# liannuaa/GenPC

Hardware: AMD Instinct MI355X
Metric: chamfer_nn_pair_dist_throughput (higher is better)
Workload: dtype f32; 1 GPU; chamfer_3DDist.forward B=1 N=M=16384 (both directions), one pair per rank; points=16384, batch=1, arith=fma

## Files before the change

### genpc_amd/csrc/chamfer.hip

```cpp
#include "nn.h"
#include "../../include/genpc_hip.h"

#include <stdlib.h>
#include <algorithm>
#include <atomic>
#include <mutex>

namespace genpc {

constexpr int kTile = 2048;




template <int R, int FMA>
__global__ __launch_bounds__(kBlock) void nn_forward_kernel(NNArgs a)
{
    __shared__ float4 tile[kTile / 4 * 3 + 3];
    const int lane = threadIdx.x & (kWave - 1);
    const int wave = threadIdx.x >> 6;
    int bid = blockIdx.x;
    const int d = (a.ndir > 1 && bid >= a.dir[1].block_begin) ? 1 : 0;
    const NNDir &D = a.dir[d];
    bid -= D.block_begin;
// ... 756 lines not shown
        NNDir &D = a.dir[d];
        D.slices = ceil_div(D.nt, a.slice_len);
        D.block_begin = (int)tb;
        D.unit_begin = units;
        tb += (long long)D.slices * b * D.qblocks;
        units += b * D.qblocks;
        if (D.slices > 1 || path == 2) {
            part += (size_t)D.slices * b * D.nq * pwords;
            any_split = true;
        }
    }
    if (tb > 0x7fffffffLL) {
        set_error("chamfer: problem too large for one launch");
        return 0;
    }
    if (any_split) {
        const size_t cnt_min = (size_t)1 << 16;
        size_t cnt_bytes = cnt_min;
        if ((size_t)units * sizeof(int) > cnt_bytes) cnt_bytes = ((size_t)units * sizeof(int) + 255) & ~(size_t)255;
        char *ws = (char *)workspace(0, cnt_bytes + part * 8, st, nullptr, cnt_min);
        if (!ws) return 0;
        if (cnt_bytes > cnt_min && !check(hipMemsetAsync(ws, 0, cnt_bytes, st), "hipMemsetAsync(arrival counters)")) return 0;
        a.arrive = (int *)ws;
        unsigned long long *wp = (unsigned long long *)(ws + cnt_bytes);
        size_t off = 0;
        for (int d = 0; d < nd; d++) {
            if (a.dir[d].slices > 1 || path == 2) {
                a.dir[d].part = wp + off;
                off += (size_t)a.dir[d].slices * b * a.dir[d].nq * pwords;
            }
        }
    }
    if (path == 2) {
        const int force = (a.debug & 2048) ? 0 : ((a.debug & 4096) ? 1 : -1);
        DedupeHint *H = dedupe_hint();
        bool own_masks = true;
        for (int d = 0; d < nd; d++) own_masks = own_masks && a.dir[d].dupmask != nullptr;
        if (force == 0) {
            for (int d = 0; d < nd; d++) a.dir[d].dupmask = nullptr;
        } else if (!own_masks) {
            long long queries = 0, targets = 0;
            for (int d = 0; d < nd; d++) { queries += (long long)b * a.dir[d].nq; targets += (long long)b * a.dir[d].nt; }
            bool run = force == 1;
            if (!run && H) {
                std::lock_guard<std::mutex> l(H->mu);
                volatile unsigned *hv = H->host;
// ... 116 lines not shown
```

### genpc_amd/csrc/nn.h

```cpp
#pragma once
#include "common.h"
#include "grid.h"

namespace genpc {

constexpr int kChunk = 32;
constexpr int kBlock = 256;
constexpr int kWavesPerBlock = kBlock / kWave;

template <int FMA>
__device__ __forceinline__ float sqdist(float dx, float dy, float dz)
{
    if (FMA) {
        float t = __fmul_rn(dy, dy);
        t = __fmaf_rn(dx, dx, t);
        return __fmaf_rn(dz, dz, t);
    } else {
        float a = __fmul_rn(dx, dx);
        float b = __fmul_rn(dy, dy);
        float c = __fmul_rn(dz, dz);
        return __fadd_rn(__fadd_rn(a, b), c);
    }
}

struct NNDir {
    const float *q;
    const float *t;
    float *out_d;
    int *out_i;
    unsigned long long *part;
    int nq, nt;
    float *tmaxp;
    const uint4 *arec;
    int ntp, ntmax;
    int fin_begin;
    const unsigned *dupmask;
    int dup_shared;
    int qblocks;
    int slices;
    int block_begin;
    int unit_begin;
};

struct NNArgs {
    NNDir dir[2];
    int ndir;
    int b;
    int slice_len;
    int *arrive;
    int debug;
    int fma;
    unsigned long long *stats;
    int hint_stride;
    unsigned *hint;
    float radius2;
};

typedef float f32x16 __attribute__((ext_vector_type(16)));

struct Top3 {
    float a1, a2, a3;
    int c1, c2;
};

__device__ __forceinline__ void top3_init(Top3 &s)
{
    s.a1 = s.a2 = s.a3 = __builtin_inff();
    s.c1 = s.c2 = -1;
}

__device__ __forceinline__ void top3_insert(Top3 &s, float m, int id)
{
    asm("v_cmp_lt_f32 vcc, %[m], %[a2]\n\t"
        "v_cndmask_b32 %[c2], %[c2], %[id], vcc\n\t"
        "v_cmp_lt_f32 vcc, %[m], %[a1]\n\t"
        "v_cndmask_b32 %[c2], %[c2], %[c1], vcc\n\t"
        "v_cndmask_b32 %[c1], %[c1], %[id], vcc\n\t"
        "v_med3_f32 %[a3], %[a2], %[a3], %[m]\n\t"
// ... 35 lines not shown
            for (int c = 7; c >= 0; c--) {
                const float dd = sqdist<FMA>(f[c * 3 + 0] - qx, f[c * 3 + 1] - qy, f[c * 3 + 2] - qz);
                const bool le = dd <= bd;
                bd = le ? dd : bd;
                bi = le ? base + c8 + c : bi;
            }
        }
    } else {
        for (int c = LEN - 1; c >= 0; c--) {
            int kk = base + c;
            kk = kk < nt ? kk : nt - 1;
            const float *tp = T + (size_t)kk * 3;
            const float dd = sqdist<FMA>(tp[0] - qx, tp[1] - qy, tp[2] - qz);
            const bool le = dd <= bd;
            bd = le ? dd : bd;
            bi = le ? kk : bi;
        }
    }
}

__device__ __forceinline__ int tile_row(int w) { return 8 * ((w >> 2) & 3) + 4 * (w >> 4) + (w & 3); }

constexpr int kRefTile = 512;
template <int FMA>
__device__ __forceinline__ void nn_exhaustive(const float *__restrict__ Qp, const float *__restrict__ T, int nt, int j,
                                              float *__restrict__ od, int *__restrict__ oi, float *s_red, int *s_fi)
{
    const int lane = threadIdx.x & (kWave - 1), wave = threadIdx.x >> 6;
    const float x = Qp[(size_t)j * 3 + 0], y = Qp[(size_t)j * 3 + 1], z = Qp[(size_t)j * 3 + 2];
    int dead = 0;
    for (int k = threadIdx.x * kRefTile; k < nt; k += kBlock * kRefTile) {
        const float *tp = T + (size_t)k * 3;
        const float hd = sqdist<FMA>(tp[0] - x, tp[1] - y, tp[2] - z);
        dead |= hd != hd;
    }
    dead = __syncthreads_or(dead);
    float bd = __builtin_inff();
    int bi = 0x7fffffff;
    if (!dead) {
        for (int k = threadIdx.x; k < nt; k += kBlock) {
            const float *tp = T + (size_t)k * 3;
            const float dd = sqdist<FMA>(tp[0] - x, tp[1] - y, tp[2] - z);
            const bool lt = dd < bd;
            bd = lt ? dd : bd;
            bi = lt ? k : bi;
        }
    } else {
        for (int k = threadIdx.x; k < nt; k += kBlock) {
            const float *hp = T + (size_t)(k & ~(kRefTile - 1)) * 3;
            const float hd = sqdist<FMA>(hp[0] - x, hp[1] - y, hp[2] - z);
            const float *tp = T + (size_t)k * 3;
            const float dd = sqdist<FMA>(tp[0] - x, tp[1] - y, tp[2] - z);
            const bool lt = dd < bd && hd == hd;
            bd = lt ? dd : bd;
            bi = lt ? k : bi;
        }
    }
#pragma unroll
    for (int o = 32; o >= 1; o >>= 1) {
        const float obd = __shfl_xor(bd, o);
        const int obi = __shfl_xor(bi, o);
        const bool other = obd < bd || (obd == bd && obi < bi);
        bd = other ? obd : bd;
        bi = other ? obi : bi;
    }
    __syncthreads();
    if (lane == 0) { s_red[wave] = bd; s_fi[wave] = bi; }
    __syncthreads();
    if (threadIdx.x == 0) {
        for (int w = 1; w < kWavesPerBlock; w++) {
            const bool other = s_red[w] < bd || (s_red[w] == bd && s_fi[w] < bi);
            bd = other ? s_red[w] : bd;
            bi = other ? s_fi[w] : bi;
        }
        const float d0 = sqdist<FMA>(T[0] - x, T[1] - y, T[2] - z);
        if (d0 != d0 || bi == 0x7fffffff) {
            bd = d0;
            bi = 0;
        }
        od[j] = bd;
        oi[j] = bi;
    }
}

__device__ __forceinline__ float nn_tau(float a_best, float qq, float tmax2, double kQT, double kTT)
{
    const double u = 1.01 * 5.9604644775390625e-8;
    const double T = sqrt((double)tmax2), qn = sqrt((double)qq);
    const double kSub = 64.0 * 1.401298464324817e-45;
    const double E1 = u * (kQT * qn * T + kTT * T * T + 3.0 * (double)qq) + kSub;
    const double eta = u * (qn + T);
    double up = (double)a_best + (double)qq + E1;
    up = sqrt(up > 0.0 ? up : 0.0) + eta;
// ... 26 lines not shown
            const float f[12] = {v[g * 3].x, v[g * 3].y, v[g * 3].z, v[g * 3].w, v[g * 3 + 1].x, v[g * 3 + 1].y,
                                 v[g * 3 + 1].z, v[g * 3 + 1].w, v[g * 3 + 2].x, v[g * 3 + 2].y, v[g * 3 + 2].z, v[g * 3 + 2].w};
#pragma unroll
            for (int c = 3; c >= 0; c--) {
                const float dd = sqdist<FMA>(f[c * 3 + 0] - qx, f[c * 3 + 1] - qy, f[c * 3 + 2] - qz);
                const bool le = dd <= bd;
                bd = le ? dd : bd;
                bi = le ? first + 4 * g + c : bi;
            }
        }
    } else {
        for (int c = 15; c >= 0; c--) {
            int kk = first + c;
            kk = kk < nt ? kk : nt - 1;
            const float *tp = T + (size_t)kk * 3;
            const float dd = sqdist<FMA>(tp[0] - qx, tp[1] - qy, tp[2] - qz);
            const bool le = dd <= bd;
            bd = le ? dd : bd;
            bi = le ? kk : bi;
        }
    }
}

int launch_nn_f16(NNArgs &a, int q, int u, int nl, int tight, long long total_blocks, hipStream_t st);
int launch_nn_finish(NNArgs &a, int nl, int upieces, float kqt, float ktt, float t2min, hipStream_t st);
int launch_nn_grid(const NNArgs &a, hipStream_t st);
size_t nn_dedupe_mask_words(int b, int n);
int launch_nn_dedupe(int b, int nclouds, const float *const pts[2], const int n[2], unsigned *const masks[2], unsigned *hint,
                     hipStream_t st);
int nn_forward(int b, int ndir, const float *q0, int n0, const float *t0, int m0, float *d0, int *i0, const float *q1,
               int n1, const float *t1, int m1, float *d1, int *i1, hipStream_t st, float radius2 = __builtin_inff(),
               const unsigned *dup0 = nullptr, const unsigned *dup1 = nullptr, int dup_shared = 0);

struct SeededGrids {
    const CellGridHdr *hdr_static, *hdr_rest;
    const int *start_static, *start_rest;
    const float4 *sorted_static, *sorted_rest;
};
size_t seeded_grids_bytes(int b, int nm, int ns);
int build_seeded_grids(int b, int nm, const float *rest_pts, int ns, const float *static_pts, void *ws, SeededGrids &g, hipStream_t st);
int launch_nn_seeded(int b, int nm, const float *moving_pts, int ns, const float *static_pts, const SeededGrids &g, const float *center,
                     int cstride, const float *params, int pstride, float *d1, int *i1, float *d2, int *i2, int fma, hipStream_t st, int sample = 1);

}
```

### genpc_amd/csrc/nn_f16.hip

```cpp
#include "nn.h"
#include <hip/hip_ext.h>
#include "../../include/genpc_hip.h"

#include <stdlib.h>

namespace genpc {

typedef _Float16 h16x8 __attribute__((ext_vector_type(8)));

#ifdef GENPC_NN_TIMELINE
__device__ unsigned long long g_timeline[4096 * 8];
#define GENPC_TL(k) do { if (threadIdx.x == 0 && blockIdx.x < 4096) { g_timeline[blockIdx.x * 8 + (k)] = __builtin_readcyclecounter(); \
    if ((k) == 0) g_timeline[blockIdx.x * 8 + 6] = wall_clock64(); if ((k) == 5) g_timeline[blockIdx.x * 8 + 7] = wall_clock64(); } } while (0)
#else
#define GENPC_TL(k) do {} while (0)
#endif
constexpr int kHTile = 1024;
constexpr double kQTh = 30.0, kTTh = 15.0;

__device__ __forceinline__ unsigned f16_bits(float v) { return (unsigned)__builtin_bit_cast(unsigned short, (_Float16)v); }

__device__ __forceinline__ unsigned split2(float v)
{
    const _Float16 h = (_Float16)v;
    const _Float16 l = (_Float16)(v - (float)h);
    return (unsigned)__builtin_bit_cast(unsigned short, h) | ((unsigned)__builtin_bit_cast(unsigned short, l) << 16);
}

__device__ __forceinline__ unsigned dup_lo(unsigned v) { return __builtin_amdgcn_perm(v, v, 0x01000100u); }
__device__ __forceinline__ unsigned dup_hi(unsigned v) { return __builtin_amdgcn_perm(v, v, 0x03020302u); }

__device__ __forceinline__ float scale_for(float m)
{
    if (!(m > 0.0f) || !(m < __builtin_inff())) return 1.0f;
    const int e = __builtin_amdgcn_frexp_expf(m);
    return __builtin_ldexpf(1.0f, 11 - e);
}

template <int Q, int U, int NL, int W, int HT, int WV>
__global__ __launch_bounds__(WV * kWave, W) void nn_f16_kernel(NNArgs a)
{
    constexpr int kThreads = WV * kWave;
    static_assert(Q >= 2, "one accumulator chain per wave violates the MFMA -> VALU wait states");
    constexpr int kC = 32 * U;
    constexpr int kRows = HT + 64;
    __shared__ uint4 plane[2][kRows];
    __shared__ float s_red[WV];
    GENPC_TL(0);
    const int lane = threadIdx.x & (kWave - 1);
    const int wave = threadIdx.x >> 6;
    const int half = lane >> 5, col = lane & 31;
    int bid = blockIdx.x;
    const int d = (a.ndir > 1 && bid >= a.dir[1].block_begin) ? 1 : 0;
    const NNDir &D = a.dir[d];
    bid -= D.block_begin;
    const int qb = bid % D.qblocks;
    const int rest = bid / D.qblocks;
    const int batch = rest % a.b;
    const int slice = rest / a.b;

    const int nq = D.nq, nt = D.nt;
    const float *__restrict__ Qp = D.q + (size_t)batch * nq * 3;
    const float *__restrict__ T = D.t + (size_t)batch * nt * 3;
    const float *cptr = a.dir[0].t + (size_t)batch * a.dir[0].nt * 3;
    const float cx = cptr[0], cy = cptr[1], cz = cptr[2];

    const int k_begin = slice * a.slice_len;
    int k_end = k_begin + a.slice_len;
    if (k_end > nt) k_end = nt;

// ... 132 lines not shown
                    float m[Q][4];
#pragma unroll
                    for (int r = 0; r < Q; r++) m[r][0] = m[r][1] = m[r][2] = m[r][3] = __builtin_inff();
#pragma unroll
                    for (int g = 0; g < U - 1; g++) {
                        if (g & 1) step(std::integral_constant<int, 1>{}, std::false_type{}, rb + 32 * g, m);
                        else step(std::integral_constant<int, 0>{}, std::false_type{}, rb + 32 * g, m);
                    }
                    if (rb + kC < tn_pad) step(std::integral_constant<int, 1>{}, std::false_type{}, rb + kC - 32, m);
                    else step(std::integral_constant<int, 1>{}, std::true_type{}, rb + kC - 32, m);
#pragma unroll
                    for (int r = 0; r < Q; r++) {
                        float v;
                        asm("v_min3_f32 %0, %1, %2, %3" : "=v"(v) : "v"(m[r][0]), "v"(m[r][1]), "v"(m[r][2]));
                        asm("v_min_f32 %0, %1, %2" : "=v"(v) : "v"(v), "v"(m[r][3]));
                        top3_insert(lst[r][n], v, t0 + rb + half);
                    }
                }
            }
        }
    }

    GENPC_TL(4);
    if (qb == 0) {
        if (nf != nf) tmax2 = __builtin_inff();
#pragma unroll
        for (int o = 32; o >= 1; o >>= 1) tmax2 = fmaxf(tmax2, __shfl_xor(tmax2, o));
        __syncthreads();
        if (lane == 0) s_red[wave] = tmax2;
        __syncthreads();
        float tm = s_red[0];
#pragma unroll
        for (int w2 = 1; w2 < WV; w2++) tm = fmaxf(tm, s_red[w2]);
        if (threadIdx.x == 0) D.tmaxp[(size_t)batch * D.slices + slice] = tm;
    }

    const size_t bnq = (size_t)a.b * nq;
    unsigned long long *P = D.part + (size_t)batch * nq;
#pragma unroll
    for (int r = 0; r < Q; r++) {
#pragma unroll
        for (int n = 0; n < NL; n++) {
            Top3 &f = lst[r][n];
            f.a1 = (f.a1 * isc) * isc;
            f.a2 = (f.a2 * isc) * isc;
            f.a3 = (f.a3 * isc) * isc;
            const float o1 = __shfl_xor(f.a1, 32), o2 = __shfl_xor(f.a2, 32), o3 = __shfl_xor(f.a3, 32);
            const int oc1 = __shfl_xor(f.c1, 32), oc2 = __shfl_xor(f.c2, 32);
            top3_insert(f, o1, oc1);
            top3_insert(f, o2, oc2);
            top3_insert(f, o3, -1);
            const int j = q0 + r * 32;
            if (!half && j < nq) {
                unsigned long long *p = P + (size_t)(slice * NL + n) * 2 * bnq + j;
                const unsigned code2 = list_enc(f.a1, f.a2);
                const unsigned code3 = list_enc(list_dec(f.a1, code2), f.a3);
                p[0] = ((unsigned long long)__float_as_uint(f.a1) << 32) | (unsigned)f.c1;
                p[bnq] = ((unsigned long long)((code2 << 16) | code3) << 32) | (unsigned)f.c2;
            }
        }
    }
    GENPC_TL(5);
}

template <int Q, int NL>
static void launch_main(const NNArgs &a, int blocks, int u, int tight, hipStream_t st, hipEvent_t e0 = nullptr, hipEvent_t e1 = nullptr)
{
#define NN_F16_LAUNCH(KERNEL, GRID, BLOCK)                                                                              \
    do {                                                                                                                \
        if (e0) hipExtLaunchKernelGGL(KERNEL, GRID, BLOCK, 0, st, e0, e1, 0, a);                                        \
        else hipLaunchKernelGGL(KERNEL, GRID, BLOCK, 0, st, a);                                                         \
    } while (0)
    const bool big = Q == 4 && tight != 1 && a.slice_len > kHTile;
    if (Q == 4 && tight == 2) {
        if (u == 2) NN_F16_LAUNCH((nn_f16_kernel<4, 2, NL, 1, 2 * kHTile, 8>), dim3(blocks), dim3(8 * kWave));
        else NN_F16_LAUNCH((nn_f16_kernel<4, 4, NL, 1, 2 * kHTile, 8>), dim3(blocks), dim3(8 * kWave));
        return;
    }
    if (big) {
        if (u == 2) NN_F16_LAUNCH((nn_f16_kernel<4, 2, NL, 2, 2 * kHTile, 4>), dim3(blocks), dim3(kBlock));
        else NN_F16_LAUNCH((nn_f16_kernel<4, 4, NL, 2, 2 * kHTile, 4>), dim3(blocks), dim3(kBlock));
        return;
    }
    if (u == 2) {
        if (tight) NN_F16_LAUNCH((nn_f16_kernel<Q, 2, NL, (Q == 4 ? 3 : 4), kHTile, 4>), dim3(blocks), dim3(kBlock));
        else NN_F16_LAUNCH((nn_f16_kernel<Q, 2, NL, (Q == 4 ? 2 : 4), kHTile, 4>), dim3(blocks), dim3(kBlock));
    } else {
        if (tight) NN_F16_LAUNCH((nn_f16_kernel<Q, 4, NL, (Q == 4 ? 3 : 4), kHTile, 4>), dim3(blocks), dim3(kBlock));
        else NN_F16_LAUNCH((nn_f16_kernel<Q, 4, NL, (Q == 4 ? 2 : 4), kHTile, 4>), dim3(blocks), dim3(kBlock));
    }
#undef NN_F16_LAUNCH
}

static thread_local bool g_prof_on = false;
static thread_local hipEvent_t g_prof_e0 = nullptr, g_prof_e1 = nullptr;

int launch_nn_f16(NNArgs &a, int q, int u, int nl, int tight, long long total_blocks, hipStream_t st)
{
    size_t bytes = 0;
    size_t off_t[2];
    for (int d = 0; d < a.ndir; d++) {
        a.dir[d].ntmax = a.dir[d].slices;
        off_t[d] = bytes;
        bytes += ((size_t)a.b * a.dir[d].ntmax * sizeof(float) + 255) & ~(size_t)255;
    }
    char *ws = (char *)workspace(9, bytes, st);
    if (!ws) return 0;
    for (int d = 0; d < a.ndir; d++) a.dir[d].tmaxp = (float *)(ws + off_t[d]);
    const int blocks = (int)total_blocks;
    hipEvent_t pe0 = nullptr, pe1 = nullptr;
    if (g_prof_on) {
        if (!g_prof_e0) { (void)hipEventCreate(&g_prof_e0); (void)hipEventCreate(&g_prof_e1); }
        pe0 = g_prof_e0;
        pe1 = g_prof_e1;
    }
    if (q == 4) {
        if (nl == 2) launch_main<4, 2>(a, blocks, u, tight, st, pe0, pe1);
        else launch_main<4, 1>(a, blocks, u, tight, st, pe0, pe1);
    } else {
        if (nl == 2) launch_main<2, 2>(a, blocks, u, 0, st, pe0, pe1);
        else launch_main<2, 1>(a, blocks, u, 0, st, pe0, pe1);
    }
    if (!check(hipGetLastError(), "nn_f16_kernel launch")) return 0;
    return launch_nn_finish(a, nl, u, (float)kQTh, (float)kTTh, 0.0f, st);
}

}

#ifdef GENPC_NN_TIMELINE
extern "C" __attribute__((visibility("default"))) int genpc_nn_timeline_read(unsigned long long *out)
{
    return hipMemcpyFromSymbol(out, HIP_SYMBOL(genpc::g_timeline), sizeof(unsigned long long) * 4096 * 8) == hipSuccess;
}
#endif

GENPC_API float genpc_nn_profile(int enable)
{
    using namespace genpc;
    float ms = -1.0f;
    if (g_prof_on && g_prof_e1 && hipEventSynchronize(g_prof_e1) == hipSuccess) (void)hipEventElapsedTime(&ms, g_prof_e0, g_prof_e1);
    g_prof_on = enable != 0;
    return ms;
}
```

### genpc_amd/csrc/nn_finish.hip

```cpp
#include "nn.h"

namespace genpc {

#ifdef GENPC_NN_TIMELINE
__device__ unsigned long long g_timeline_fin[4096 * 8];
#define GENPC_TLF(k) do { if (threadIdx.x == 0 && blockIdx.x < 4096) g_timeline_fin[blockIdx.x * 8 + (k)] = __builtin_readcyclecounter(); } while (0)
#else
#define GENPC_TLF(k) do {} while (0)
#endif

constexpr int kFQ = 64;
constexpr int kFWork = 2048;

template <int FMA>
__global__ __launch_bounds__(kBlock) void nn_finish_kernel(NNArgs a, int nl, int upieces, float kqt, float ktt, float t2min)
{
    __shared__ unsigned long long s_best[kFQ];
    __shared__ float4 s_q[kFQ];
    __shared__ float s_a[4][kFQ];
    __shared__ int s_c[4][kFQ];
    __shared__ int s_qflag[kFQ];
    __shared__ int s_flagged[kFQ];
    __shared__ unsigned s_work[kFWork];
    __shared__ float s_red[kWavesPerBlock];
    __shared__ int s_fi[kWavesPerBlock];
    __shared__ int s_misc[3];
    GENPC_TLF(0);
    const int lane = threadIdx.x & (kWave - 1), wave = threadIdx.x >> 6;
    int bid = blockIdx.x;
    const int d = (a.ndir > 1 && bid >= a.dir[1].fin_begin) ? 1 : 0;
    const NNDir &D = a.dir[d];
    bid -= D.fin_begin;
    const int nq = D.nq, nt = D.nt;
    const int fblocks = (nq + kFQ - 1) / kFQ;
    const int batch = bid / fblocks, fb = bid % fblocks;
    const float *__restrict__ Qp = D.q + (size_t)batch * nq * 3;
    const float *__restrict__ T = D.t + (size_t)batch * nt * 3;
    float *__restrict__ od = D.out_d + (size_t)batch * nq;
    int *__restrict__ oi = D.out_i + (size_t)batch * nq;
    const size_t bnq = (size_t)a.b * nq;
    const unsigned long long *P = D.part + (size_t)batch * nq;
    const int nlists = D.slices * nl;

    const int ql = threadIdx.x & (kFQ - 1), part = threadIdx.x >> 6;
    int j = fb * kFQ + ql;
    const bool live = j < nq;
    j = live ? j : nq - 1;

    const float *cptr = a.dir[0].t + (size_t)batch * a.dir[0].nt * 3;
    const float ccx = cptr[0], ccy = cptr[1], ccz = cptr[2];
    unsigned long long w0[kMaxLists / 4], w1[kMaxLists / 4];
    float amin = __builtin_inff();
#pragma unroll
    for (int k = 0; k < kMaxLists / 4; k++) {
        const int li = part + 4 * k;
        w0[k] = 0x7f800000ull << 32;
        w1[k] = 0xff00ff00ull << 32;
        if (li < nlists) {
            const unsigned long long *p = P + (size_t)li * 2 * bnq + j;
            w0[k] = p[0];
            w1[k] = p[bnq];
        }
    }
    int cmin = -1, kmin = -1;
#pragma unroll
    for (int k = 0; k < kMaxLists / 4; k++) {
        const float a1 = __uint_as_float((unsigned)(w0[k] >> 32));
        if (a1 < amin) { amin = a1; cmin = (int)(unsigned)w0[k]; kmin = k; }
    }
    s_a[part][ql] = amin;
    s_c[part][ql] = cmin;
    float tmax2 = 0.0f;
    {
        const float *tp = D.tmaxp + (size_t)batch * D.ntmax;
        for (int i = threadIdx.x; i < D.ntmax; i += kBlock) tmax2 = fmaxf(tmax2, tp[i]);
#pragma unroll
        for (int o = 32; o >= 1; o >>= 1) tmax2 = fmaxf(tmax2, __shfl_xor(tmax2, o));
        if (lane == 0) s_red[wave] = tmax2;
    }
    if (part == 0) {
        s_q[ql] = make_float4(Qp[(size_t)j * 3 + 0], Qp[(size_t)j * 3 + 1], Qp[(size_t)j * 3 + 2], 0.0f);
        s_best[ql] = ~0ull;
        s_qflag[ql] = 0;
    }
    if (threadIdx.x == 0) { s_misc[0] = 0; s_misc[1] = 0; s_misc[2] = 0; }
    __syncthreads();
    GENPC_TLF(1);
    tmax2 = fmaxf(fmaxf(s_red[0], s_red[1]), fmaxf(s_red[2], s_red[3]));
    int bp = 0;
    float abest = s_a[0][ql];
#pragma unroll
    for (int q2 = 1; q2 < 4; q2++) {
        const float v = s_a[q2][ql];
        if (v < abest) { abest = v; bp = q2; }
    }
    const int cb = s_c[bp][ql];
    const float4 qv = s_q[ql];
    unsigned long long mine = ~0ull;
    int pieces = 0;
    if (cb >= 0 && live && !(a.debug & 1)) {
        const int h = cb & 1, c0 = cb & ~1;
        const int left = (nt - c0 + 31) >> 5;
        const int n2 = left < upieces ? left : upieces;
        if (part < n2) {
            float dd;
            int ii;
            rescan_half<FMA>(T, nt, c0 + 32 * part, h, qv.x, qv.y, qv.z, dd, ii);
            mine = ((unsigned long long)__float_as_uint(dd) << 32) | (unsigned)ii;
            pieces = 1;
        }
    }
    float tau, qq;
    {
        const float x = qv.x - ccx, y = qv.y - ccy, z = qv.z - ccz;
        qq = __fmaf_rn(z, z, __fmaf_rn(y, y, __fmul_rn(x, x)));
        tau = nn_tau(abest, qq, tmax2, (double)kqt, (double)ktt);
        if (!(tmax2 >= t2min)) tau = __builtin_nanf("");
        if (!(tmax2 < __builtin_inff()) || !(qq < __builtin_inff())) tau = __builtin_nanf("");
        if (a.debug & 16) tau = __builtin_inff();
    }
    if (mine != ~0ull) atomicMin(&s_best[ql], mine);
    GENPC_TLF(2);
    bool flag = (a.debug & 8) != 0 || !(tau == tau);
    int ncand = 0;
    auto consider = [&](float av, int c, bool is_best) {
        if (av <= tau) {
            ncand++;
            if (c < 0) {
                flag = true;
            } else if (live && !is_best) {
                const int h = c & 1, c0 = c & ~1;
                const int left = (nt - c0 + 31) >> 5;
                const int n2 = left < upieces ? left : upieces;
                const int w = atomicAdd(&s_misc[0], n2);
                if (w + n2 <= kFWork) {
                    for (int k = 0; k < n2; k++) s_work[w + k] = ((unsigned)ql << 22) | (unsigned)((((c0 >> 5) + k) << 1) | h);
                } else {
                    flag = true;
                }
            }
        }
    };
#pragma unroll
    for (int k = 0; k < kMaxLists / 4; k++) {
        const float a1 = __uint_as_float((unsigned)(w0[k] >> 32));
        const unsigned codes = (unsigned)(w1[k] >> 32);
        const float a2 = list_dec(a1, codes >> 16), a3 = list_dec(a2, codes & 0xffffu);
        if (!(a3 > tau)) flag = true;
        consider(a1, (int)(unsigned)w0[k], part == bp && k == kmin);
        consider(a2, (int)(unsigned)w1[k], false);
    }
    if (flag && live) s_qflag[ql] = 1;
    if (a.debug & 32) {
        __syncthreads();
        if (part == 0) s_a[0][ql] = 0.0f;
        __syncthreads();
        atomicAdd(&s_a[0][ql], (float)ncand);
        __syncthreads();
        if (part == 0 && live) { od[j] = abest + qq; oi[j] = (int)s_a[0][ql] | (s_qflag[ql] ? 1 << 16 : 0); }
        return;
    }
    __syncthreads();
    GENPC_TLF(3);
    const int nwork = min(s_misc[0], kFWork);
    if (nwork > 0 && !(a.debug & 1)) {
        for (int w = threadIdx.x; w < nwork; w += kBlock) {
            const unsigned it = s_work[w];
            const int slot = (int)(it >> 22);
            const float4 qs = s_q[slot];
            float dd;
            int ii;
            rescan_half<FMA>(T, nt, (int)((it & 0x3fffffu) >> 1) << 5, (int)(it & 1u), qs.x, qs.y, qs.z, dd, ii);
            atomicMin(&s_best[slot], ((unsigned long long)__float_as_uint(dd) << 32) | (unsigned)ii);
            pieces++;
        }
        __syncthreads();
    }
    if (a.stats && pieces) atomicAdd(&s_misc[2], pieces);
    __syncthreads();
    GENPC_TLF(4);
    if (part == 0 && live) {
        if (s_qflag[ql]) {
            s_flagged[atomicAdd(&s_misc[1], 1)] = j;
        } else {
            const unsigned long long v = s_best[ql];
            od[j] = __uint_as_float((unsigned)(v >> 32));
            oi[j] = (int)(unsigned)v;
        }
    }
    __syncthreads();
    const int nflag = s_misc[1];
    if (nflag && a.hint && threadIdx.x == 0 && blockIdx.x % a.hint_stride == 0 && !(tmax2 != tmax2) && tmax2 < __builtin_inff())
        __hip_atomic_fetch_add(a.hint, (unsigned)(nflag * a.hint_stride), __ATOMIC_RELAXED, __HIP_MEMORY_SCOPE_SYSTEM);
    if (a.stats && threadIdx.x == 0) {
        atomicAdd(&a.stats[0], (unsigned long long)min(kFQ, nq - fb * kFQ));
        atomicAdd(&a.stats[1], (unsigned long long)nflag);
        atomicAdd(&a.stats[2], (unsigned long long)s_misc[2]);
    }
    for (int fidx = 0; fidx < nflag; fidx++) nn_exhaustive<FMA>(Qp, T, nt, s_flagged[fidx], od, oi, s_red, s_fi);
    GENPC_TLF(5);
}

int launch_nn_finish(NNArgs &a, int nl, int upieces, float kqt, float ktt, float t2min, hipStream_t st)
{
    long long fb = 0;
    for (int d = 0; d < a.ndir; d++) {
        a.dir[d].fin_begin = (int)fb;
        fb += (long long)a.b * ceil_div(a.dir[d].nq, kFQ);
    }
    if (fb > 0x7fffffffLL) {
        set_error("chamfer: problem too large for one launch");
        return 0;
    }
    a.hint_stride = (int)ceil_div64(fb, 16);
    if (a.fma)
        hipLaunchKernelGGL((nn_finish_kernel<1>), dim3((unsigned)fb), dim3(kBlock), 0, st, a, nl, upieces, kqt, ktt, t2min);
    else
        hipLaunchKernelGGL((nn_finish_kernel<0>), dim3((unsigned)fb), dim3(kBlock), 0, st, a, nl, upieces, kqt, ktt, t2min);
    return check(hipGetLastError(), "nn_finish_kernel launch") ? 1 : 0;
}

}

#ifdef GENPC_NN_TIMELINE
extern "C" __attribute__((visibility("default"))) int genpc_nn_timeline_read_finish(unsigned long long *out)
{
    return hipMemcpyFromSymbol(out, HIP_SYMBOL(genpc::g_timeline_fin), sizeof(unsigned long long) * 4096 * 8) == hipSuccess;
}
#endif
```

Before: 17720 Gpair-dist/s.

## Fuse finish pass into f16 NN kernel via cooperative slice arrival

Moves the per-query finish step (candidate rescan, threshold check, exhaustive fallback) into a shared device function. The wide 8-wave f16 search kernel now runs it in place once all slices of a query block have arrived, using a bounded spin wait on an arrival counter and reusing the staging shared memory. Finished runs are marked in a run_done array so the separate finish kernel exits early for them, which is meant to cut the second launch's work and its global round trip. In exchange it adds atomic stores and loads and spin-waiting inside the search kernel, and it depends on the timing of slice co-residency, falling back to the old finish path when the wait times out.

New measurement: 15730 Gpair-dist/s. 0.888x the previous value.

```diff
diff --git a/genpc_amd/csrc/chamfer.hip b/genpc_amd/csrc/chamfer.hip
--- a/genpc_amd/csrc/chamfer.hip
+++ b/genpc_amd/csrc/chamfer.hip
@@ -802,6 +802,10 @@
         if (!ws) return 0;
         if (cnt_bytes > cnt_min && !check(hipMemsetAsync(ws, 0, cnt_bytes, st), "hipMemsetAsync(arrival counters)")) return 0;
         a.arrive = (int *)ws;
+        if (wide && !(a.debug & 32) && (size_t)units * (2 + kRunsPerUnit) * sizeof(int) <= cnt_min) {
+            a.sib_done = a.arrive + units;
+            a.run_done = a.arrive + 2 * units;
+        }
         unsigned long long *wp = (unsigned long long *)(ws + cnt_bytes);
         size_t off = 0;
         for (int d = 0; d < nd; d++) {
diff --git a/genpc_amd/csrc/nn.h b/genpc_amd/csrc/nn.h
--- a/genpc_amd/csrc/nn.h
+++ b/genpc_amd/csrc/nn.h
@@ -40,6 +40,7 @@
     int slices;
     int block_begin;
     int unit_begin;
+    float *tmaxu;
 };
 
 struct NNArgs {
@@ -54,6 +55,8 @@
     int hint_stride;
     unsigned *hint;
     float radius2;
+    int *sib_done;
+    int *run_done;
 };
 
 typedef float f32x16 __attribute__((ext_vector_type(16)));
@@ -135,14 +138,14 @@
 __device__ __forceinline__ int tile_row(int w) { return 8 * ((w >> 2) & 3) + 4 * (w >> 4) + (w & 3); }
 
 constexpr int kRefTile = 512;
-template <int FMA>
+template <int FMA, int NT = kBlock>
 __device__ __forceinline__ void nn_exhaustive(const float *__restrict__ Qp, const float *__restrict__ T, int nt, int j,
                                               float *__restrict__ od, int *__restrict__ oi, float *s_red, int *s_fi)
 {
     const int lane = threadIdx.x & (kWave - 1), wave = threadIdx.x >> 6;
     const float x = Qp[(size_t)j * 3 + 0], y = Qp[(size_t)j * 3 + 1], z = Qp[(size_t)j * 3 + 2];
     int dead = 0;
-    for (int k = threadIdx.x * kRefTile; k < nt; k += kBlock * kRefTile) {
+    for (int k = threadIdx.x * kRefTile; k < nt; k += NT * kRefTile) {
         const float *tp = T + (size_t)k * 3;
         const float hd = sqdist<FMA>(tp[0] - x, tp[1] - y, tp[2] - z);
         dead |= hd != hd;
@@ -151,7 +154,7 @@
     float bd = __builtin_inff();
     int bi = 0x7fffffff;
     if (!dead) {
-        for (int k = threadIdx.x; k < nt; k += kBlock) {
+        for (int k = threadIdx.x; k < nt; k += NT) {
             const float *tp = T + (size_t)k * 3;
             const float dd = sqdist<FMA>(tp[0] - x, tp[1] - y, tp[2] - z);
             const bool lt = dd < bd;
@@ -159,7 +162,7 @@
             bi = lt ? k : bi;
         }
     } else {
-        for (int k = threadIdx.x; k < nt; k += kBlock) {
+        for (int k = threadIdx.x; k < nt; k += NT) {
             const float *hp = T + (size_t)(k & ~(kRefTile - 1)) * 3;
             const float hd = sqdist<FMA>(hp[0] - x, hp[1] - y, hp[2] - z);
             const float *tp = T + (size_t)k * 3;
@@ -181,7 +184,7 @@
     if (lane == 0) { s_red[wave] = bd; s_fi[wave] = bi; }
     __syncthreads();
     if (threadIdx.x == 0) {
-        for (int w = 1; w < kWavesPerBlock; w++) {
+        for (int w = 1; w < NT / kWave; w++) {
             const bool other = s_red[w] < bd || (s_red[w] == bd && s_fi[w] < bi);
             bd = other ? s_red[w] : bd;
             bi = other ? s_fi[w] : bi;
@@ -254,7 +257,212 @@
     }
 }
 
+constexpr int kFQ = 64;
+constexpr int kFWork = 2048;
+constexpr int kRunsPerUnit = 16;
+
+struct FinishGroup {
+    float4 q[kFQ];
+    unsigned long long best[kFQ];
+    float a[4][kFQ];
+    int c[4][kFQ];
+    int qflag[kFQ];
+    int flagged[kFQ];
+    unsigned work[kFWork];
+    float red[kWavesPerBlock];
+    int misc[4];
+};
+
+#ifndef GENPC_TLF
+#define GENPC_TLF(k) do {} while (0)
+#endif
+
+template <int FMA, int G>
+__device__ __forceinline__ void nn_finish_body(const NNArgs &a, const NNDir &D, int batch, int fb, bool active, FinishGroup *FG,
+                                               float *x_red, int *x_fi, const float *tmaxv, int ntmax, int vblock, int nl,
+                                               int upieces, float kqt, float ktt, float t2min)
+{
+    const int tg = threadIdx.x & (kBlock - 1);
+    FinishGroup &S = FG[G > 1 ? threadIdx.x / kBlock : 0];
+    const int lane = threadIdx.x & (kWave - 1);
+    const int nq = D.nq, nt = D.nt;
+    const float *__restrict__ Qp = D.q + (size_t)batch * nq * 3;
+    const float *__restrict__ T = D.t + (size_t)batch * nt * 3;
+    float *__restrict__ od = D.out_d + (size_t)batch * nq;
+    int *__restrict__ oi = D.out_i + (size_t)batch * nq;
+    const size_t bnq = (size_t)a.b * nq;
+    const unsigned long long *P = D.part + (size_t)batch * nq;
+    const int nlists = D.slices * nl;
+
+    const int ql = tg & (kFQ - 1), part = tg >> 6;
+    int j = (active ? fb : 0) * kFQ + ql;
+    const bool live = active && j < nq;
+    j = j < nq ? j : nq - 1;
+
+    const float *cptr = a.dir[0].t + (size_t)batch * a.dir[0].nt * 3;
+    const float ccx = cptr[0], ccy = cptr[1], ccz = cptr[2];
+    unsigned long long w0[kMaxLists / 4], w1[kMaxLists / 4];
+    float amin = __builtin_inff();
+#pragma unroll
+    for (int k = 0; k < kMaxLists / 4; k++) {
+        const int li = part + 4 * k;
+        w0[k] = 0x7f800000ull << 32;
+        w1[k] = 0xff00ff00ull << 32;
+        if (li < nlists) {
+            const unsigned long long *p = P + (size_t)li * 2 * bnq + j;
+            if (G > 1) {
+                w0[k] = __hip_atomic_load(p, __ATOMIC_RELAXED, __HIP_MEMORY_SCOPE_AGENT);
+                w1[k] = __hip_atomic_load(p + bnq, __ATOMIC_RELAXED, __HIP_MEMORY_SCOPE_AGENT);
+            } else {
+                w0[k] = p[0];
+                w1[k] = p[bnq];
+            }
+        }
+    }
+    int cmin = -1, kmin = -1;
+#pragma unroll
+    for (int k = 0; k < kMaxLists / 4; k++) {
+        const float a1 = __uint_as_float((unsigned)(w0[k] >> 32));
+        if (a1 < amin) { amin = a1; cmin = (int)(unsigned)w0[k]; kmin = k; }
+    }
+    S.a[part][ql] = amin;
+    S.c[part][ql] = cmin;
+    float tmax2 = 0.0f;
+    {
+        for (int i = tg; i < ntmax; i += kBlock)
+            tmax2 = fmaxf(tmax2, G > 1 ? __hip_atomic_load(tmaxv + i, __ATOMIC_RELAXED, __HIP_MEMORY_SCOPE_AGENT) : tmaxv[i]);
+#pragma unroll
+        for (int o = 32; o >= 1; o >>= 1) tmax2 = fmaxf(tmax2, __shfl_xor(tmax2, o));
+        if (lane == 0) S.red[part] = tmax2;
+    }
+    if (part == 0) {
+        S.q[ql] = make_float4(Qp[(size_t)j * 3 + 0], Qp[(size_t)j * 3 + 1], Qp[(size_t)j * 3 + 2], 0.0f);
+        S.best[ql] = ~0ull;
+        S.qflag[ql] = 0;
+    }
+    if (tg == 0) { S.misc[0] = 0; S.misc[1] = 0; S.misc[2] = 0; }
+    __syncthreads();
+    GENPC_TLF(1);
+    tmax2 = fmaxf(fmaxf(S.red[0], S.red[1]), fmaxf(S.red[2], S.red[3]));
+    int bp = 0;
+    float abest = S.a[0][ql];
+#pragma unroll
+    for (int q2 = 1; q2 < 4; q2++) {
+        const float v = S.a[q2][ql];
+        if (v < abest) { abest = v; bp = q2; }
+    }
+    const int cb = S.c[bp][ql];
+    const float4 qv = S.q[ql];
+    unsigned long long mine = ~0ull;
+    int pieces = 0;
+    if (cb >= 0 && live && !(a.debug & 1)) {
+        const int h = cb & 1, c0 = cb & ~1;
+        const int left = (nt - c0 + 31) >> 5;
+        const int n2 = left < upieces ? left : upieces;
+        if (part < n2) {
+            float dd;
+            int ii;
+            rescan_half<FMA>(T, nt, c0 + 32 * part, h, qv.x, qv.y, qv.z, dd, ii);
+            mine = ((unsigned long long)__float_as_uint(dd) << 32) | (unsigned)ii;
+            pieces = 1;
+        }
+    }
+    float tau, qq;
+    {
+        const float x = qv.x - ccx, y = qv.y - ccy, z = qv.z - ccz;
+        qq = __fmaf_rn(z, z, __fmaf_rn(y, y, __fmul_rn(x, x)));
+        tau = nn_tau(abest, qq, tmax2, (double)kqt, (double)ktt);
+        if (!(tmax2 >= t2min)) tau = __builtin_nanf("");
+        if (!(tmax2 < __builtin_inff()) || !(qq < __builtin_inff())) tau = __builtin_nanf("");
+        if (a.debug & 16) tau = __builtin_inff();
+    }
+    if (mine != ~0ull) atomicMin(&S.best[ql], mine);
+    GENPC_TLF(2);
+    bool flag = (a.debug & 8) != 0 || !(tau == tau);
+    int ncand = 0;
+    auto consider = [&](float av, int c, bool is_best) {
+        if (av <= tau) {
+            ncand++;
+            if (c < 0) {
+                flag = true;
+            } else if (live && !is_best) {
+                const int h = c & 1, c0 = c & ~1;
+                const int left = (nt - c0 + 31) >> 5;
+                const int n2 = left < upieces ? left : upieces;
+                const int w = atomicAdd(&S.misc[0], n2);
+                if (w + n2 <= kFWork) {
+                    for (int k = 0; k < n2; k++) S.work[w + k] = ((unsigned)ql << 22) | (unsigned)((((c0 >> 5) + k) << 1) | h);
+                } else {
+                    flag = true;
+                }
+            }
+        }
+    };
+#pragma unroll
+    for (int k = 0; k < kMaxLists / 4; k++) {
+        const float a1 = __uint_as_float((unsigned)(w0[k] >> 32));
+        const unsigned codes = (unsigned)(w1[k] >> 32);
+        const float a2 = list_dec(a1, codes >> 16), a3 = list_dec(a2, codes & 0xffffu);
+        if (!(a3 > tau)) flag = true;
+        consider(a1, (int)(unsigned)w0[k], part == bp && k == kmin);
+        consider(a2, (int)(unsigned)w1[k], false);
+    }
+    if (flag && live) S.qflag[ql] = 1;
+    if (G == 1 && (a.debug & 32)) {
+        __syncthreads();
+        if (part == 0) S.a[0][ql] = 0.0f;
+        __syncthreads();
+        atomicAdd(&S.a[0][ql], (float)ncand);
+        __syncthreads();
+        if (part == 0 && live) { od[j] = abest + qq; oi[j] = (int)S.a[0][ql] | (S.qflag[ql] ? 1 << 16 : 0); }
+        return;
+    }
+    __syncthreads();
+    GENPC_TLF(3);
+    const int nwork = min(S.misc[0], kFWork);
+    if (!(a.debug & 1)) {
+        for (int w = tg; w < nwork; w += kBlock) {
+            const unsigned it = S.work[w];
+            const int slot = (int)(it >> 22);
+            const float4 qs = S.q[slot];
+            float dd;
+            int ii;
+            rescan_half<FMA>(T, nt, (int)((it & 0x3fffffu) >> 1) << 5, (int)(it & 1u), qs.x, qs.y, qs.z, dd, ii);
+            atomicMin(&S.best[slot], ((unsigned long long)__float_as_uint(dd) << 32) | (unsigned)ii);
+            pieces++;
+        }
+    }
+    if (a.stats && pieces) atomicAdd(&S.misc[2], pieces);
+    __syncthreads();
+    GENPC_TLF(4);
+    if (part == 0 && live) {
+        if (S.qflag[ql]) {
+            S.flagged[atomicAdd(&S.misc[1], 1)] = j;
+        } else {
+            const unsigned long long v = S.best[ql];
+            od[j] = __uint_as_float((unsigned)(v >> 32));
+            oi[j] = (int)(unsigned)v;
+        }
+    }
+    __syncthreads();
+    const int nflag = S.misc[1];
+    if (nflag && a.hint && tg == 0 && vblock % a.hint_stride == 0 && !(tmax2 != tmax2) && tmax2 < __builtin_inff())
+        __hip_atomic_fetch_add(a.hint, (unsigned)(nflag * a.hint_stride), __ATOMIC_RELAXED, __HIP_MEMORY_SCOPE_SYSTEM);
+    if (a.stats && tg == 0 && active) {
+        if (G > 1 || !(a.debug & 128)) atomicAdd(&a.stats[0], (unsigned long long)min(kFQ, nq - fb * kFQ));
+        atomicAdd(&a.stats[1], (unsigned long long)nflag);
+        atomicAdd(&a.stats[2], (unsigned long long)S.misc[2]);
+    }
+#pragma unroll
+    for (int g = 0; g < G; g++) {
+        const int nf = FG[g].misc[1];
+        for (int fidx = 0; fidx < nf; fidx++) nn_exhaustive<FMA, G * kBlock>(Qp, T, nt, FG[g].flagged[fidx], od, oi, x_red, x_fi);
+    }
+    GENPC_TLF(5);
+}
+
 int launch_nn_f16(NNArgs &a, int q, int u, int nl, int tight, long long total_blocks, hipStream_t st);
+long long nn_finish_layout(NNArgs &a);
 int launch_nn_finish(NNArgs &a, int nl, int upieces, float kqt, float ktt, float t2min, hipStream_t st);
 int launch_nn_grid(const NNArgs &a, hipStream_t st);
 size_t nn_dedupe_mask_words(int b, int n);
diff --git a/genpc_amd/csrc/nn_f16.hip b/genpc_amd/csrc/nn_f16.hip
--- a/genpc_amd/csrc/nn_f16.hip
+++ b/genpc_amd/csrc/nn_f16.hip
@@ -12,8 +12,14 @@
 __device__ unsigned long long g_timeline[4096 * 8];
 #define GENPC_TL(k) do { if (threadIdx.x == 0 && blockIdx.x < 4096) { g_timeline[blockIdx.x * 8 + (k)] = __builtin_readcyclecounter(); \
     if ((k) == 0) g_timeline[blockIdx.x * 8 + 6] = wall_clock64(); if ((k) == 5) g_timeline[blockIdx.x * 8 + 7] = wall_clock64(); } } while (0)
+__device__ unsigned long long g_timeline_coop[4096 * 8];
+#define GENPC_TLC(k) do { if (threadIdx.x == 0 && blockIdx.x < 4096) g_timeline_coop[blockIdx.x * 8 + (k)] = wall_clock64(); } while (0)
+#define GENPC_TLC_INFO(unit, ok) do { if (blockIdx.x < 4096) { g_timeline_coop[blockIdx.x * 8 + 3] = (unsigned long long)(unit) + 1; \
+    g_timeline_coop[blockIdx.x * 8 + 4] = (unsigned long long)(ok); } } while (0)
 #else
 #define GENPC_TL(k) do {} while (0)
+#define GENPC_TLC(k) do {} while (0)
+#define GENPC_TLC_INFO(unit, ok) do {} while (0)
 #endif
 constexpr int kHTile = 1024;
 constexpr double kQTh = 30.0, kTTh = 15.0;
@@ -37,7 +43,9 @@
     return __builtin_ldexpf(1.0f, 11 - e);
 }
 
-template <int Q, int U, int NL, int W, int HT, int WV>
+constexpr unsigned long long kCoopWaitTicks = 2000;
+
+template <int Q, int U, int NL, int W, int HT, int WV, int FMA>
 __global__ __launch_bounds__(WV * kWave, W) void nn_f16_kernel(NNArgs a)
 {
     constexpr int kThreads = WV * kWave;
@@ -46,6 +54,8 @@
     constexpr int kRows = HT + 64;
     __shared__ uint4 plane[2][kRows];
     __shared__ float s_red[WV];
+    __shared__ int s_coop;
+    const bool coop = WV == 8 && a.run_done != nullptr;
     GENPC_TL(0);
     const int lane = threadIdx.x & (kWave - 1);
     const int wave = threadIdx.x >> 6;
@@ -224,7 +234,7 @@
     }
 
     GENPC_TL(4);
-    if (qb == 0) {
+    if (qb == 0 || coop) {
         if (nf != nf) tmax2 = __builtin_inff();
 #pragma unroll
         for (int o = 32; o >= 1; o >>= 1) tmax2 = fmaxf(tmax2, __shfl_xor(tmax2, o));
@@ -234,7 +244,9 @@
         float tm = s_red[0];
 #pragma unroll
         for (int w2 = 1; w2 < WV; w2++) tm = fmaxf(tm, s_red[w2]);
-        if (threadIdx.x == 0) D.tmaxp[(size_t)batch * D.slices + slice] = tm;
+        if (threadIdx.x == 0 && qb == 0) D.tmaxp[(size_t)batch * D.slices + slice] = tm;
+        if (threadIdx.x == 0 && coop)
+            __hip_atomic_store(D.tmaxu + ((size_t)batch * D.qblocks + qb) * D.slices + slice, tm, __ATOMIC_RELAXED, __HIP_MEMORY_SCOPE_AGENT);
     }
 
     const size_t bnq = (size_t)a.b * nq;
@@ -257,12 +269,70 @@
                 unsigned long long *p = P + (size_t)(slice * NL + n) * 2 * bnq + j;
                 const unsigned code2 = list_enc(f.a1, f.a2);
                 const unsigned code3 = list_enc(list_dec(f.a1, code2), f.a3);
-                p[0] = ((unsigned long long)__float_as_uint(f.a1) << 32) | (unsigned)f.c1;
-                p[bnq] = ((unsigned long long)((code2 << 16) | code3) << 32) | (unsigned)f.c2;
+                const unsigned long long v0 = ((unsigned long long)__float_as_uint(f.a1) << 32) | (unsigned)f.c1;
+                const unsigned long long v1 = ((unsigned long long)((code2 << 16) | code3) << 32) | (unsigned)f.c2;
+                if (WV == 8) {
+                    __hip_atomic_store(p, v0, __ATOMIC_RELAXED, __HIP_MEMORY_SCOPE_AGENT);
+                    __hip_atomic_store(p + bnq, v1, __ATOMIC_RELAXED, __HIP_MEMORY_SCOPE_AGENT);
+                } else {
+                    p[0] = v0;
+                    p[bnq] = v1;
+                }
             }
         }
     }
     GENPC_TL(5);
+
+    if constexpr (WV == 8) {
+        if (coop) {
+            const int unit = D.unit_begin + batch * D.qblocks + qb;
+            asm volatile("s_waitcnt vmcnt(0)" ::: "memory");
+            __syncthreads();
+            if (threadIdx.x == 0) {
+                int *cnt = a.arrive + unit;
+                GENPC_TLC(0);
+                __hip_atomic_fetch_add(cnt, 1, __ATOMIC_RELAXED, __HIP_MEMORY_SCOPE_AGENT);
+                int ok = 0;
+                if (!(a.debug & 64)) {
+                    const unsigned long long w0 = wall_clock64();
+                    for (;;) {
+                        if (__hip_atomic_load(cnt, __ATOMIC_RELAXED, __HIP_MEMORY_SCOPE_AGENT) == D.slices) { ok = 1; break; }
+                        if (wall_clock64() - w0 > kCoopWaitTicks) break;
+                        __builtin_amdgcn_s_sleep(4);
+                    }
+                }
+                s_coop = ok;
+                GENPC_TLC(1);
+                GENPC_TLC_INFO(unit, ok);
+            }
+            __syncthreads();
+            if (s_coop) {
+                static_assert(2 * sizeof(FinishGroup) + 16 * sizeof(float) <= sizeof(plane), "finish state must fit the staging planes");
+                FinishGroup *FG = reinterpret_cast<FinishGroup *>(&plane[0][0]);
+                float *x_red = reinterpret_cast<float *>(FG + 2);
+                int *x_fi = reinterpret_cast<int *>(x_red + 8);
+                const int fblocks = (nq + kFQ - 1) / kFQ;
+                const int group = threadIdx.x / kBlock;
+                const float *tmaxv = D.tmaxu + ((size_t)batch * D.qblocks + qb) * D.slices;
+                for (int r = slice; r < kRunsPerUnit / 2 && (qb * kRunsPerUnit + 2 * r) * kFQ < nq; r += D.slices) {
+                    const int fb = qb * kRunsPerUnit + 2 * r + group;
+                    const bool active = fb < fblocks;
+                    nn_finish_body<FMA, 2>(a, D, batch, fb, active, FG, x_red, x_fi, tmaxv, D.slices, D.fin_begin + batch * fblocks + fb,
+                                           NL, U, (float)kQTh, (float)kTTh, 0.0f);
+                    __syncthreads();
+                    if (active && (threadIdx.x & (kBlock - 1)) == 0) a.run_done[(size_t)unit * kRunsPerUnit + 2 * r + group] = 1;
+                }
+            }
+            GENPC_TLC(2);
+            if (threadIdx.x == 0) {
+                int *sd = a.sib_done + unit;
+                if (__hip_atomic_fetch_add(sd, 1, __ATOMIC_RELAXED, __HIP_MEMORY_SCOPE_AGENT) == D.slices - 1) {
+                    __hip_atomic_store(a.arrive + unit, 0, __ATOMIC_RELAXED, __HIP_MEMORY_SCOPE_AGENT);
+                    __hip_atomic_store(sd, 0, __ATOMIC_RELAXED, __HIP_MEMORY_SCOPE_AGENT);
+                }
+            }
+        }
+    }
 }
 
 template <int Q, int NL>
@@ -275,21 +345,26 @@
     } while (0)
     const bool big = Q == 4 && tight != 1 && a.slice_len > kHTile;
     if (Q == 4 && tight == 2) {
-        if (u == 2) NN_F16_LAUNCH((nn_f16_kernel<4, 2, NL, 1, 2 * kHTile, 8>), dim3(blocks), dim3(8 * kWave));
-        else NN_F16_LAUNCH((nn_f16_kernel<4, 4, NL, 1, 2 * kHTile, 8>), dim3(blocks), dim3(8 * kWave));
+        if (a.fma) {
+            if (u == 2) NN_F16_LAUNCH((nn_f16_kernel<4, 2, NL, 1, 2 * kHTile, 8, 1>), dim3(blocks), dim3(8 * kWave));
+            else NN_F16_LAUNCH((nn_f16_kernel<4, 4, NL, 1, 2 * kHTile, 8, 1>), dim3(blocks), dim3(8 * kWave));
+        } else {
+            if (u == 2) NN_F16_LAUNCH((nn_f16_kernel<4, 2, NL, 1, 2 * kHTile, 8, 0>), dim3(blocks), dim3(8 * kWave));
+            else NN_F16_LAUNCH((nn_f16_kernel<4, 4, NL, 1, 2 * kHTile, 8, 0>), dim3(blocks), dim3(8 * kWave));
+        }
         return;
     }
     if (big) {
-        if (u == 2) NN_F16_LAUNCH((nn_f16_kernel<4, 2, NL, 2, 2 * kHTile, 4>), dim3(blocks), dim3(kBlock));
-        else NN_F16_LAUNCH((nn_f16_kernel<4, 4, NL, 2, 2 * kHTile, 4>), dim3(blocks), dim3(kBlock));
+        if (u == 2) NN_F16_LAUNCH((nn_f16_kernel<4, 2, NL, 2, 2 * kHTile, 4, 0>), dim3(blocks), dim3(kBlock));
+        else NN_F16_LAUNCH((nn_f16_kernel<4, 4, NL, 2, 2 * kHTile, 4, 0>), dim3(blocks), dim3(kBlock));
         return;
     }
     if (u == 2) {
-        if (tight) NN_F16_LAUNCH((nn_f16_kernel<Q, 2, NL, (Q == 4 ? 3 : 4), kHTile, 4>), dim3(blocks), dim3(kBlock));
-        else NN_F16_LAUNCH((nn_f16_kernel<Q, 2, NL, (Q == 4 ? 2 : 4), kHTile, 4>), dim3(blocks), dim3(kBlock));
+        if (tight) NN_F16_LAUNCH((nn_f16_kernel<Q, 2, NL, (Q == 4 ? 3 : 4), kHTile, 4, 0>), dim3(blocks), dim3(kBlock));
+        else NN_F16_LAUNCH((nn_f16_kernel<Q, 2, NL, (Q == 4 ? 2 : 4), kHTile, 4, 0>), dim3(blocks), dim3(kBlock));
     } else {
-        if (tight) NN_F16_LAUNCH((nn_f16_kernel<Q, 4, NL, (Q == 4 ? 3 : 4), kHTile, 4>), dim3(blocks), dim3(kBlock));
-        else NN_F16_LAUNCH((nn_f16_kernel<Q, 4, NL, (Q == 4 ? 2 : 4), kHTile, 4>), dim3(blocks), dim3(kBlock));
+        if (tight) NN_F16_LAUNCH((nn_f16_kernel<Q, 4, NL, (Q == 4 ? 3 : 4), kHTile, 4, 0>), dim3(blocks), dim3(kBlock));
+        else NN_F16_LAUNCH((nn_f16_kernel<Q, 4, NL, (Q == 4 ? 2 : 4), kHTile, 4, 0>), dim3(blocks), dim3(kBlock));
     }
 #undef NN_F16_LAUNCH
 }
@@ -306,10 +381,21 @@
         off_t[d] = bytes;
         bytes += ((size_t)a.b * a.dir[d].ntmax * sizeof(float) + 255) & ~(size_t)255;
     }
+    size_t off_u[2] = {0, 0};
+    if (a.run_done) {
+        for (int d = 0; d < a.ndir; d++) {
+            off_u[d] = bytes;
+            bytes += ((size_t)a.b * a.dir[d].qblocks * a.dir[d].slices * sizeof(float) + 255) & ~(size_t)255;
+        }
+    }
     char *ws = (char *)workspace(9, bytes, st);
     if (!ws) return 0;
-    for (int d = 0; d < a.ndir; d++) a.dir[d].tmaxp = (float *)(ws + off_t[d]);
+    for (int d = 0; d < a.ndir; d++) {
+        a.dir[d].tmaxp = (float *)(ws + off_t[d]);
+        a.dir[d].tmaxu = a.run_done ? (float *)(ws + off_u[d]) : nullptr;
+    }
     const int blocks = (int)total_blocks;
+    if (nn_finish_layout(a) <= 0) return 0;
     hipEvent_t pe0 = nullptr, pe1 = nullptr;
     if (g_prof_on) {
         if (!g_prof_e0) { (void)hipEventCreate(&g_prof_e0); (void)hipEventCreate(&g_prof_e1); }
@@ -334,6 +420,10 @@
 {
     return hipMemcpyFromSymbol(out, HIP_SYMBOL(genpc::g_timeline), sizeof(unsigned long long) * 4096 * 8) == hipSuccess;
 }
+extern "C" __attribute__((visibility("default"))) int genpc_nn_timeline_read_coop(unsigned long long *out)
+{
+    return hipMemcpyFromSymbol(out, HIP_SYMBOL(genpc::g_timeline_coop), sizeof(unsigned long long) * 4096 * 8) == hipSuccess;
+}
 #endif
 
 GENPC_API float genpc_nn_profile(int enable)
diff --git a/genpc_amd/csrc/nn_finish.hip b/genpc_amd/csrc/nn_finish.hip
--- a/genpc_amd/csrc/nn_finish.hip
+++ b/genpc_amd/csrc/nn_finish.hip
@@ -1,207 +1,38 @@
+#ifdef GENPC_NN_TIMELINE
+namespace genpc { __device__ unsigned long long g_timeline_fin[4096 * 8]; }
+#define GENPC_TLF(k) do { if (threadIdx.x == 0 && blockIdx.x < 4096) g_timeline_fin[blockIdx.x * 8 + (k)] = __builtin_readcyclecounter(); } while (0)
+#endif
 #include "nn.h"
 
 namespace genpc {
 
-#ifdef GENPC_NN_TIMELINE
-__device__ unsigned long long g_timeline_fin[4096 * 8];
-#define GENPC_TLF(k) do { if (threadIdx.x == 0 && blockIdx.x < 4096) g_timeline_fin[blockIdx.x * 8 + (k)] = __builtin_readcyclecounter(); } while (0)
-#else
-#define GENPC_TLF(k) do {} while (0)
-#endif
-
-constexpr int kFQ = 64;
-constexpr int kFWork = 2048;
-
 template <int FMA>
 __global__ __launch_bounds__(kBlock) void nn_finish_kernel(NNArgs a, int nl, int upieces, float kqt, float ktt, float t2min)
 {
-    __shared__ unsigned long long s_best[kFQ];
-    __shared__ float4 s_q[kFQ];
-    __shared__ float s_a[4][kFQ];
-    __shared__ int s_c[4][kFQ];
-    __shared__ int s_qflag[kFQ];
-    __shared__ int s_flagged[kFQ];
-    __shared__ unsigned s_work[kFWork];
+    __shared__ FinishGroup s_group;
     __shared__ float s_red[kWavesPerBlock];
     __shared__ int s_fi[kWavesPerBlock];
-    __shared__ int s_misc[3];
     GENPC_TLF(0);
-    const int lane = threadIdx.x & (kWave - 1), wave = threadIdx.x >> 6;
     int bid = blockIdx.x;
     const int d = (a.ndir > 1 && bid >= a.dir[1].fin_begin) ? 1 : 0;
     const NNDir &D = a.dir[d];
     bid -= D.fin_begin;
-    const int nq = D.nq, nt = D.nt;
-    const int fblocks = (nq + kFQ - 1) / kFQ;
+    const int fblocks = (D.nq + kFQ - 1) / kFQ;
     const int batch = bid / fblocks, fb = bid % fblocks;
-    const float *__restrict__ Qp = D.q + (size_t)batch * nq * 3;
-    const float *__restrict__ T = D.t + (size_t)batch * nt * 3;
-    float *__restrict__ od = D.out_d + (size_t)batch * nq;
-    int *__restrict__ oi = D.out_i + (size_t)batch * nq;
-    const size_t bnq = (size_t)a.b * nq;
-    const unsigned long long *P = D.part + (size_t)batch * nq;
-    const int nlists = D.slices * nl;
-
-    const int ql = threadIdx.x & (kFQ - 1), part = threadIdx.x >> 6;
-    int j = fb * kFQ + ql;
-    const bool live = j < nq;
-    j = live ? j : nq - 1;
-
-    const float *cptr = a.dir[0].t + (size_t)batch * a.dir[0].nt * 3;
-    const float ccx = cptr[0], ccy = cptr[1], ccz = cptr[2];
-    unsigned long long w0[kMaxLists / 4], w1[kMaxLists / 4];
-    float amin = __builtin_inff();
-#pragma unroll
-    for (int k = 0; k < kMaxLists / 4; k++) {
-        const int li = part + 4 * k;
-        w0[k] = 0x7f800000ull << 32;
-        w1[k] = 0xff00ff00ull << 32;
-        if (li < nlists) {
-            const unsigned long long *p = P + (size_t)li * 2 * bnq + j;
-            w0[k] = p[0];
-            w1[k] = p[bnq];
+    if (a.run_done) {
+        int *dw = a.run_done + (size_t)(D.unit_begin + batch * D.qblocks + fb / kRunsPerUnit) * kRunsPerUnit + fb % kRunsPerUnit;
+        const int done = __hip_atomic_load(dw, __ATOMIC_RELAXED, __HIP_MEMORY_SCOPE_AGENT);
+        __syncthreads();
+        if (done) {
+            if (threadIdx.x == 0) *dw = 0;
+            return;
         }
     }
-    int cmin = -1, kmin = -1;
-#pragma unroll
-    for (int k = 0; k < kMaxLists / 4; k++) {
-        const float a1 = __uint_as_float((unsigned)(w0[k] >> 32));
-        if (a1 < amin) { amin = a1; cmin = (int)(unsigned)w0[k]; kmin = k; }
-    }
-    s_a[part][ql] = amin;
-    s_c[part][ql] = cmin;
-    float tmax2 = 0.0f;
-    {
-        const float *tp = D.tmaxp + (size_t)batch * D.ntmax;
-        for (int i = threadIdx.x; i < D.ntmax; i += kBlock) tmax2 = fmaxf(tmax2, tp[i]);
-#pragma unroll
-        for (int o = 32; o >= 1; o >>= 1) tmax2 = fmaxf(tmax2, __shfl_xor(tmax2, o));
-        if (lane == 0) s_red[wave] = tmax2;
-    }
-    if (part == 0) {
-        s_q[ql] = make_float4(Qp[(size_t)j * 3 + 0], Qp[(size_t)j * 3 + 1], Qp[(size_t)j * 3 + 2], 0.0f);
-        s_best[ql] = ~0ull;
-        s_qflag[ql] = 0;
-    }
-    if (threadIdx.x == 0) { s_misc[0] = 0; s_misc[1] = 0; s_misc[2] = 0; }
-    __syncthreads();
-    GENPC_TLF(1);
-    tmax2 = fmaxf(fmaxf(s_red[0], s_red[1]), fmaxf(s_red[2], s_red[3]));
-    int bp = 0;
-    float abest = s_a[0][ql];
-#pragma unroll
-    for (int q2 = 1; q2 < 4; q2++) {
-        const float v = s_a[q2][ql];
-        if (v < abest) { abest = v; bp = q2; }
-    }
-    const int cb = s_c[bp][ql];
-    const float4 qv = s_q[ql];
-    unsigned long long mine = ~0ull;
-    int pieces = 0;
-    if (cb >= 0 && live && !(a.debug & 1)) {
-        const int h = cb & 1, c0 = cb & ~1;
-        const int left = (nt - c0 + 31) >> 5;
-        const int n2 = left < upieces ? left : upieces;
-        if (part < n2) {
-            float dd;
-            int ii;
-            rescan_half<FMA>(T, nt, c0 + 32 * part, h, qv.x, qv.y, qv.z, dd, ii);
-            mine = ((unsigned long long)__float_as_uint(dd) << 32) | (unsigned)ii;
-            pieces = 1;
-        }
-    }
-    float tau, qq;
-    {
-        const float x = qv.x - ccx, y = qv.y - ccy, z = qv.z - ccz;
-        qq = __fmaf_rn(z, z, __fmaf_rn(y, y, __fmul_rn(x, x)));
-        tau = nn_tau(abest, qq, tmax2, (double)kqt, (double)ktt);
-        if (!(tmax2 >= t2min)) tau = __builtin_nanf("");
-        if (!(tmax2 < __builtin_inff()) || !(qq < __builtin_inff())) tau = __builtin_nanf("");
-        if (a.debug & 16) tau = __builtin_inff();
-    }
-    if (mine != ~0ull) atomicMin(&s_best[ql], mine);
-    GENPC_TLF(2);
-    bool flag = (a.debug & 8) != 0 || !(tau == tau);
-    int ncand = 0;
-    auto consider = [&](float av, int c, bool is_best) {
-        if (av <= tau) {
-            ncand++;
-            if (c < 0) {
-                flag = true;
-            } else if (live && !is_best) {
-                const int h = c & 1, c0 = c & ~1;
-                const int left = (nt - c0 + 31) >> 5;
-                const int n2 = left < upieces ? left : upieces;
-                const int w = atomicAdd(&s_misc[0], n2);
-                if (w + n2 <= kFWork) {
-                    for (int k = 0; k < n2; k++) s_work[w + k] = ((unsigned)ql << 22) | (unsigned)((((c0 >> 5) + k) << 1) | h);
-                } else {
-                    flag = true;
-                }
-            }
-        }
-    };
-#pragma unroll
-    for (int k = 0; k < kMaxLists / 4; k++) {
-        const float a1 = __uint_as_float((unsigned)(w0[k] >> 32));
-        const unsigned codes = (unsigned)(w1[k] >> 32);
-        const float a2 = list_dec(a1, codes >> 16), a3 = list_dec(a2, codes & 0xffffu);
-        if (!(a3 > tau)) flag = true;
-        consider(a1, (int)(unsigned)w0[k], part == bp && k == kmin);
-        consider(a2, (int)(unsigned)w1[k], false);
-    }
-    if (flag && live) s_qflag[ql] = 1;
-    if (a.debug & 32) {
-        __syncthreads();
-        if (part == 0) s_a[0][ql] = 0.0f;
-        __syncthreads();
-        atomicAdd(&s_a[0][ql], (float)ncand);
-        __syncthreads();
-        if (part == 0 && live) { od[j] = abest + qq; oi[j] = (int)s_a[0][ql] | (s_qflag[ql] ? 1 << 16 : 0); }
-        return;
-    }
-    __syncthreads();
-    GENPC_TLF(3);
-    const int nwork = min(s_misc[0], kFWork);
-    if (nwork > 0 && !(a.debug & 1)) {
-        for (int w = threadIdx.x; w < nwork; w += kBlock) {
-            const unsigned it = s_work[w];
-            const int slot = (int)(it >> 22);
-            const float4 qs = s_q[slot];
-            float dd;
-            int ii;
-            rescan_half<FMA>(T, nt, (int)((it & 0x3fffffu) >> 1) << 5, (int)(it & 1u), qs.x, qs.y, qs.z, dd, ii);
-            atomicMin(&s_best[slot], ((unsigned long long)__float_as_uint(dd) << 32) | (unsigned)ii);
-            pieces++;
-        }
-        __syncthreads();
-    }
-    if (a.stats && pieces) atomicAdd(&s_misc[2], pieces);
-    __syncthreads();
-    GENPC_TLF(4);
-    if (part == 0 && live) {
-        if (s_qflag[ql]) {
-            s_flagged[atomicAdd(&s_misc[1], 1)] = j;
-        } else {
-            const unsigned long long v = s_best[ql];
-            od[j] = __uint_as_float((unsigned)(v >> 32));
-            oi[j] = (int)(unsigned)v;
-        }
-    }
-    __syncthreads();
-    const int nflag = s_misc[1];
-    if (nflag && a.hint && threadIdx.x == 0 && blockIdx.x % a.hint_stride == 0 && !(tmax2 != tmax2) && tmax2 < __builtin_inff())
-        __hip_atomic_fetch_add(a.hint, (unsigned)(nflag * a.hint_stride), __ATOMIC_RELAXED, __HIP_MEMORY_SCOPE_SYSTEM);
-    if (a.stats && threadIdx.x == 0) {
-        atomicAdd(&a.stats[0], (unsigned long long)min(kFQ, nq - fb * kFQ));
-        atomicAdd(&a.stats[1], (unsigned long long)nflag);
-        atomicAdd(&a.stats[2], (unsigned long long)s_misc[2]);
-    }
-    for (int fidx = 0; fidx < nflag; fidx++) nn_exhaustive<FMA>(Qp, T, nt, s_flagged[fidx], od, oi, s_red, s_fi);
-    GENPC_TLF(5);
+    nn_finish_body<FMA, 1>(a, D, batch, fb, true, &s_group, s_red, s_fi, D.tmaxp + (size_t)batch * D.ntmax, D.ntmax, (int)blockIdx.x, nl,
+                           upieces, kqt, ktt, t2min);
 }
 
-int launch_nn_finish(NNArgs &a, int nl, int upieces, float kqt, float ktt, float t2min, hipStream_t st)
+long long nn_finish_layout(NNArgs &a)
 {
     long long fb = 0;
     for (int d = 0; d < a.ndir; d++) {
@@ -213,6 +44,13 @@
         return 0;
     }
     a.hint_stride = (int)ceil_div64(fb, 16);
+    return fb;
+}
+
+int launch_nn_finish(NNArgs &a, int nl, int upieces, float kqt, float ktt, float t2min, hipStream_t st)
+{
+    const long long fb = nn_finish_layout(a);
+    if (fb <= 0) return 0;
     if (a.fma)
         hipLaunchKernelGGL((nn_finish_kernel<1>), dim3((unsigned)fb), dim3(kBlock), 0, st, a, nl, upieces, kqt, ktt, t2min);
     else
```
